# TORlN/HDR-to-SDR

Hardware: AMD Instinct MI355X
Metric: Mpixel/s HDR10->SDR (4K frames) at 1/2/4/8 GPUs; % HBM roofline (higher is better)
Workload: dtype f32

## Files before the change

hdr-to-sdr_amd/csrc/h2s_api.hip:

```cpp
#include <stdio.h>
#include <stdlib.h>

#include "h2s_host.h"

using namespace h2s::host;
using h2s::FastParams;
using h2s::KParams;

namespace {
thread_local std::string g_err;
}

namespace h2s {
namespace host {

int fail(h2s_ctx* c, int code, const std::string& msg) {
  if (c) c->err = msg;
  else g_err = msg;
  return code;
}

int hip_fail(h2s_ctx* c, hipError_t e, const char* what) {
  return fail(c, H2S_E_HIP, std::string(what) + ": " + hipGetErrorString(e));
}
// ... 129 lines not shown
  hipError_t e = hipSuccess;
  for (Event& ev : c->pend) {
    const hipError_t r = hipEventSynchronize(ev.ev);
    if (e == hipSuccess) e = r;
    c->ev_free.push_back(std::move(ev));
  }
  c->pend.clear();
  if (e != hipSuccess) return hip_fail(c, e, "draining queued launches");
  return 0;
}

int aux_stream(h2s_ctx* c, hipStream_t* out) {
  if (int rc = c->aux.get(c, "table stream")) return rc;
  *out = c->d_lut.pool = c->d_lut_yuv.pool = c->d_lut8x.pool = c->aux.s;
  return 0;
}

static hipError_t table_copy(h2s_ctx* c, void* dst, const void* src, size_t bytes) {
  hipError_t e = hipMemcpyAsync(dst, src, bytes, hipMemcpyHostToDevice, c->aux.s);
  return e == hipSuccess ? hipStreamSynchronize(c->aux.s) : e;
}

int upload_table(h2s_ctx* c, DevBuf& buf, const void* src, size_t bytes, const char* what) {
  if (int rc = buf.reserve(c, bytes, what)) return rc;
  hipError_t e = table_copy(c, buf.p, src, bytes);
  return e == hipSuccess ? 0 : hip_fail(c, e, (std::string(what) + " upload").c_str());
}

int note_launch(h2s_ctx* c, hipStream_t s) {
  if (c->pend.size() >= 32) {
    size_t j = 0;
    for (size_t i = 0; i < c->pend.size(); i++) {
      if (hipEventQuery(c->pend[i].ev) == hipSuccess) c->ev_free.push_back(std::move(c->pend[i]));
      else c->pend[j++] = std::move(c->pend[i]);
    }
    c->pend.resize(j);
  }
  Event ev;
  if (!c->ev_free.empty()) {
    ev = std::move(c->ev_free.back());
    c->ev_free.pop_back();
  }
  if (int rc = ev.get(c, "launch event")) return rc;
  hipError_t e = hipEventRecord(ev.ev, s);
  if (e != hipSuccess) {
    c->ev_free.push_back(std::move(ev));
    return hip_fail(c, e, "launch event");
  }
  c->pend.push_back(std::move(ev));
  return 0;
}

int queued_exit(h2s_ctx* c, hipStream_t s, int rc) {
  const std::string msg = c->err;
  if (note_launch(c, s) != 0) (void)hipStreamSynchronize(s);
  c->err = msg;
  return rc;
}

static int ensure_lut8x(h2s_ctx* c, hipStream_t s) {
  if (c->d_lut8x && c->lut8x_ok) return 0;
  hipStream_t aux;
  bool grew = false;
  int rc;
  if ((rc = aux_stream(c, &aux)) || (rc = c->d_lut8x.reserve(c, sizeof(unsigned) << 24, "lut3d 8-bit table", &grew)))
    return rc;
  if (grew && hipStreamSynchronize(aux) != hipSuccess) {
    c->d_lut8x.release();
    return fail(c, H2S_E_OOM, "lut3d 8-bit table allocation failed");
  }
  hipError_t e = h2s::build_lut8x(c->d_lut, c->lut_n, c->d_lut8x, s);
  if (e != hipSuccess) return hip_fail(c, e, "lut3d 8-bit table build");
  if ((rc = c->lut_built.mark(c, s, "lut3d 8-bit table build"))) return rc;
  c->lut8x_ok = true;
  return 0;
}

static int ensure_lut_yuv(h2s_ctx* c, const KParams& k, hipStream_t s) {
  int rc;
  if ((rc = c->lut_built.wait(c, s, "lattice build ordering"))) return rc;
  if (k.rgba8) return ensure_lut8x(c, s);
  if (c->d_lut_yuv && c->lut_yuv_scale == k.qscale && c->lut_yuv_rgb == k.rgba8) return 0;
  const size_t cnt = (size_t)c->lut_n * c->lut_n * c->lut_n;
  const size_t pad = 12 * (1 + (size_t)c->lut_n + (size_t)c->lut_n * c->lut_n) + 16;
  hipStream_t aux;
  bool grew = false;
  if ((rc = aux_stream(c, &aux)) || (rc = c->d_lut_yuv.reserve(c, cnt * 3 * sizeof(float) + pad, "YUV lattice", &grew)))
    return rc;
  if (grew) {
    hipError_t e = hipMemsetAsync(c->d_lut_yuv + cnt * 3, 0, pad, aux);
    if (e == hipSuccess) e = hipStreamSynchronize(aux);
    if (e != hipSuccess) {
      c->d_lut_yuv.release();
      return fail(c, H2S_E_OOM, "YUV lattice allocation failed");
    }
  }
  h2s::YuvLutConsts K;
  K.s = k.qscale;
  K.rgb = k.rgba8;
  for (int i = 0; i < 3; i++) K.k709[i] = k.k709[i], K.kcb[i] = k.kcb[i], K.kcr[i] = k.kcr[i];
  hipError_t e = h2s::build_lut_yuv(c->d_lut, c->d_lut_yuv, c->lut_n, K, s);
  if (e != hipSuccess) return hip_fail(c, e, "YUV lattice build");
  if ((rc = c->lut_built.mark(c, s, "YUV lattice build"))) return rc;
  c->lut_yuv_scale = k.qscale;
  c->lut_yuv_rgb = k.rgba8;
  return 0;
}

int prepare(h2s_ctx* c, KParams* k, bool need_lut) {
  if (!c->params_set) return fail(c, H2S_E_INVALID_ARG, "h2s_set_params was not called");
  if (need_lut && c->params.lut_enabled && !c->d_lut)
    return fail(c, H2S_E_LUT_MISSING, "lut_enabled but no LUT loaded (h2s_set_lut)");
  *k = c->k;
  k->lut = c->d_lut;
  k->lut_n = c->lut_n;
  k->lut_sg = c->lut_n;
  k->lut_sb = c->lut_n * c->lut_n;
  k->lut_max = (float)(c->lut_n - 1);
  k->eq_lut = c->d_eq;
  k->dovi = c->dovi_n ? (const h2s::DoviRec*)c->d_dovi : nullptr;
  k->dovi_n = c->dovi_n, k->dovi_f0 = 0;
  return 0;
}

KParams frame_range(const KParams& k, int f0, int n) {
  KParams kf = k;
  for (int p = 0; p < 3; p++) {
    kf.in[p] += (long long)f0 * kf.in_fp[p];
    kf.out[p] += (long long)f0 * kf.out_fp[p];
  }
  kf.nframes = n;
  kf.total = (long long)n * kf.ch * kf.ngx;
  kf.dovi_f0 += f0;
  return kf;
}

static int tiled_width(const KParams& k) { return k.W & ~(h2s::TBW - 1); }

static h2s::TileKey tile_key_of(const KParams& k, bool dbg) {
  return h2s::tile_key(k, k.in_cstep == 2 || k.out_cstep == 2, dbg);
}

hipError_t launch_tiles(const h2s_ctx* c, const KParams& k, const Route& r, const TileOpts& o) {
  FastParams F;
  resolve_fast(c, k, &F);
  for (int p = 0; p < 3; p++) {
    F.in[p] = k.in[p], F.in_ls[p] = k.in_ls[p], F.in_fp[p] = k.in_fp[p];
    F.out[p] = k.out[p], F.out_ls[p] = k.out_ls[p], F.out_fp[p] = k.out_fp[p];
  }
  F.W = tiled_width(k), F.H = k.H, F.cw = k.cw, F.ch = k.ch;
  F.icw = k.icw, F.ich = k.ich;
  F.chroma_edge = k.chroma_edge;
  F.in_semi = k.in_cstep == 2, F.in_sh = k.in_sh, F.out_semi = k.out_cstep == 2, F.out_sh = k.out_sh;
  for (int p = 0; p < 3; p++) {
    const long long ib = (long long)(p ? k.ich : k.H) * k.in_ls[p], ob = (long long)(p ? k.ch : k.H) * k.out_ls[p];
    F.in_bytes[p] = (int)(ib < 0x7fffffff ? ib : 0x7fffffff);
    F.out_bytes[p] = (int)(ob < 0x7fffffff ? ob : 0x7fffffff);
  }
  F.nbx = (unsigned)(F.W / h2s::TBW);
  F.nby = (unsigned)((k.H + h2s::TBH - 1) / h2s::TBH);
  F.nframes = (unsigned)k.nframes;
  F.tpb = c->tiles_per_block;
  F.cv_frames = o.cv_frames;
  F.dbg = o.dbg_out;
  F.dbg_stage = o.dbg;
  F.dbg_w = k.W;
  F.dbg_lut = c->d_lut;
  F.inv_nm1 = 1.0f / (float)(c->lut_n - 1);
  F.chr444 = o.chr444;
  F.chr_w = k.W;
  F.inv_c56 = 1.0f / F.c56;
  F.dovi = k.dovi, F.dovi_n = k.dovi_n, F.dovi_f0 = k.dovi_f0;
  if (k.dovi) {
// ... 533 lines not shown
```

hdr-to-sdr_amd/csrc/h2s_fast.hip:

```cpp
#include <hip/hip_runtime.h>

#include "h2s_tile_sets.h"

H2S_TILE_UNIT(fast)

namespace h2s {

__global__ void k_build_lut_yuv(const float4* rgb, float* yuv, int n3, const YuvLutConsts K) {
  const int i = blockIdx.x * 256 + threadIdx.x;
  if (i >= n3) return;
  const float4 c = rgb[i];
  const float R = clamp01(c.x), G = clamp01(c.y), B = clamp01(c.z);
  const float Y = K.k709[0] * R + K.k709[1] * G + K.k709[2] * B;
  const float cb = K.kcb[0] * R + K.kcb[1] * G + K.kcb[2] * B;
  const float cr = K.kcr[0] * R + K.kcr[1] * G + K.kcr[2] * B;
  const float s = K.s;
  if (K.rgb) {
    yuv[3 * i] = c.x, yuv[3 * i + 1] = c.y, yuv[3 * i + 2] = c.z;
    return;
  }
  constexpr float Y_ROUND = 0.0f;
  yuv[3 * i] = (16.0f + 219.0f * Y) * s + Y_ROUND;
  yuv[3 * i + 1] = 224.0f * s * 0.25f * cb;
  yuv[3 * i + 2] = 224.0f * s * 0.25f * cr;
}

TileKey tile_key(const KParams& k, bool semi, bool dbg) {
  TileKey t;
  t.trc = k.dovi ? 2 : k.transfer;
  t.tm = k.tonemap;
  t.lp = k.pipe == PIPE_LIBPLACEBO ? 1 : 0;
  t.desat = !k.desat_on ? 0 : (k.lr == 1.0f && k.lg == 1.0f && k.lb == 1.0f ? 2 : 1);
  if (t.tm == 7 || t.tm == 8 || t.lp) t.desat = 0;
  t.dbg = dbg ? 1 : 0;
  t.sub = k.vco ? 3 : k.sub;
  t.semi = semi || t.sub ? 1 : 0;
  return t;
}

namespace {

struct TileSet {
  int dbg, lp, semi, sub, family;
  hipError_t (*launch)(const FastParams&, const TileKey&, dim3, size_t, hipStream_t);
};
const TileSet SETS[] = {
#define S(UNIT, DBG, LP, SEMI, SUB, FAMILY) {DBG, LP, SEMI, SUB, FAMILY_##FAMILY, launch_set<SET_##UNIT>},
    H2S_TILE_SETS(S)
#undef S
};

const TileSet* set_of(const TileKey& k) {
  for (const TileSet& r : SETS)
    if (r.dbg == k.dbg && r.lp == k.lp && r.semi == k.semi && r.sub == k.sub && family_case(r.family, k)) return &r;
  return nullptr;
}

}

bool tile_instance(const TileKey& k) { return set_of(k) != nullptr; }

hipError_t launch_fast(const FastParams& F, const TileKey& k, hipStream_t s) {
  const long long nt = (long long)F.nbx * F.nby * F.nframes;
  if (nt == 0) return hipSuccess;
  const long long nb = (nt + F.tpb - 1) / F.tpb;
  dim3 grid((unsigned)nb);
  const size_t lds = ((size_t)F.eq_n * sizeof(uint16_t) + 15) & ~(size_t)15;
  const TileSet* set = set_of(k);
  return set ? set->launch(F, k, grid, lds, s) : hipErrorInvalidValue;
}

hipError_t build_lut_yuv(const float4* rgb, float* yuv, int n, const YuvLutConsts& K, hipStream_t st) {
  const int n3 = n * n * n;
  hipLaunchKernelGGL(k_build_lut_yuv, dim3((n3 + 255) / 256), dim3(256), 0, st, rgb, yuv, n3, K);
  return hipGetLastError();
}

}
```

hdr-to-sdr_amd/csrc/h2s_host.h:

```cpp
#pragma once
#include <hip/hip_runtime.h>
#include <math.h>
#include <stdint.h>
#include <string.h>

#include <algorithm>
#include <string>
#include <vector>

#define H2S_PRIVATE_TEST_HOOKS
#include "../../include/h2s.h"
#include "h2s_launch.h"
#include "h2s_params.h"
#include "h2s_peak.h"
#include "h2s_srcprev.h"

#pragma GCC visibility push(hidden)

namespace h2s {
namespace host {

constexpr int kEvRing = 256;
constexpr int kMaxChunks = 8;

// ... 72 lines not shown
    std::swap(ev, o.ev);
    return *this;
  }
  ~Event() {
    if (ev) hipEventDestroy(ev);
  }
  int get(h2s_ctx* c, const char* what, unsigned flags = hipEventDisableTiming) {
    if (ev) return 0;
    hipError_t e = hipEventCreateWithFlags(&ev, flags);
    if (e == hipSuccess) return 0;
    ev = nullptr;
    return hip_fail(c, e, what);
  }
};

struct Ordered {
  Event ev;
  bool pending = false;
  int wait(h2s_ctx* c, hipStream_t s, const char* what) {
    if (!pending) return 0;
    if (hipEventQuery(ev.ev) == hipSuccess) {
      pending = false;
      return 0;
    }
    hipError_t e = hipStreamWaitEvent(s, ev.ev, 0);
    return e == hipSuccess ? 0 : hip_fail(c, e, what);
  }
  int mark(h2s_ctx* c, hipStream_t s, const char* what) {
    if (int rc = ev.get(c, what)) return rc;
    hipError_t e = hipEventRecord(ev.ev, s);
    if (e != hipSuccess) return hip_fail(c, e, what);
    pending = true;
    return 0;
  }
  int sync_host(h2s_ctx* c, const char* what) {
    if (!pending) return 0;
    hipError_t e = hipEventSynchronize(ev.ev);
    if (e != hipSuccess) return hip_fail(c, e, what);
    pending = false;
    return 0;
  }
};

struct ScaleTaps {
  enum Axis { X, Y, CX, CY };
  int W = 0, H = 0, ow = 0, oh = 0;
  int T[4] = {0, 0, 0, 0};
  size_t woff[4] = {0, 0, 0, 0}, soff[4] = {0, 0, 0, 0};
  std::vector<float> w;
  std::vector<int> s;
  Dev<float> d_w;
  Dev<int> d_s;
  long long uploads = 0;
  const float* wt(int a) const { return d_w + woff[a]; }
  const int* st(int a) const { return d_s + soff[a]; }
};

}
}

struct h2s_ctx {
  int device = 0;
  h2s_params params{};
  bool params_set = false;
  h2s::KParams k{};
  h2s::host::Stream aux;
  h2s::host::Dev<float4> d_lut;
  int lut_n = 0;
  bool lut_unit = false;
  h2s::host::Dev<float> d_lut_yuv;
  float lut_yuv_scale = -1.0f;
  int lut_yuv_rgb = 0;
  h2s::host::Dev<unsigned> d_lut8x;
  bool lut8x_ok = false;
  h2s::host::Ordered lut_built;
  bool fast_enabled = true;
  bool lp_exact = false;
  h2s::host::Format in_fmt = h2s::host::PLANAR_420, out_fmt = h2s::host::PLANAR_420;
  h2s::host::Dev<h2s::DoviRec> d_dovi;
  int dovi_n = 0;
  bool dovi_tile = false;
  int peak_blocks = h2s::PEAK_BLOCKS;
  bool serial_host = false;
  int tiles_per_block = 8;
  h2s::host::Dev<uint16_t> d_eq;
  h2s::host::Dev<float4> d_pq;
  h2s::host::Dev<float4> d_hlg;
  h2s::host::Dev<float4> d_pqi;
  h2s::host::Dev<uint8_t> d_stage;
  h2s::host::Dev<uint8_t> d_prev;
  h2s::host::Dev<float2> d_stats;
  int stats_nf = 0;
  h2s::host::Dev<double2> d_fstat;
  h2s::host::Dev<h2s::CurveConsts> d_curve;
  h2s::host::Dev<h2s::PeakState> d_pk;
  h2s::host::Ordered peak_use;
  int peak_chunk = 0;
  h2s::host::Stream pk_s[2];
  std::vector<h2s::host::Event> pk_ev;
  std::string err;
  bool fail_after_launch = false;
  bool timing = false;
  h2s::host::Event ev0[h2s::host::kEvRing], ev1[h2s::host::kEvRing];
  long long ev_count = 0;
  h2s::host::Stream ps[3];
  h2s::host::Event pev[2 * h2s::host::kMaxChunks + 2];
  std::vector<h2s::host::Event> pend, ev_free;
  h2s::host::Dev<float2> d_chr;
  h2s::host::Ordered chr_use;
  h2s::host::Dev<uint8_t> d_scale;
  h2s::host::ScaleTaps scale_taps;
  h2s::host::Ordered scale_use;
};

namespace h2s {
namespace host {

struct DeviceGuard {
  int prev = -1;
  explicit DeviceGuard(int dev) {
    if (hipGetDevice(&prev) != hipSuccess) prev = -1;
    if (prev != dev) hipSetDevice(dev);
  }
  ~DeviceGuard() {
    int cur = -1;
    if (prev >= 0 && hipGetDevice(&cur) == hipSuccess && cur != prev) hipSetDevice(prev);
  }
};

struct Route {
  int path;
  bool vec, out8;
  Format in_fmt, out_fmt;
  hipStream_t s;
  bool tile() const { return path == H2S_PATH_TILE || path == H2S_PATH_TILE_TAIL; }
  Route on(hipStream_t other) const {
    Route r = *this;
    r.s = other;
    return r;
  }
};

struct TileOpts {
  const CurveConsts* cv_frames = nullptr;
  int dbg = 0;
  float* dbg_out = nullptr;
  float2* chr444 = nullptr;
};

enum Columns { COLUMNS_ALL, COLUMNS_RAGGED };


struct SourceConsts {
  double y_scale, y_off, y_black;
  double c_scale, c_off, mid;
  double m_rcr, m_gcb, m_gcr, m_bcb;
};
SourceConsts source_consts(int bits, bool full, int matrix = H2S_SRC_MATRIX_BT2020NC);
void source_kparams(KParams* k, int bits, bool full);

int validate_params(h2s_ctx* c, const h2s_params* p);
void resolve(const h2s_params* p, KParams* k, std::vector<uint16_t>* eq);
void resolve_fast(const h2s_ctx* c, const KParams& k, FastParams* F);
void build_pqi_table(std::vector<float4>* out);
void build_pq_table(double scale, std::vector<float4>* out);
void build_hlg_table(std::vector<float4>* out);
void chroma_taps(float* wx7, float* wy8);
// ... 41 lines not shown
```

hdr-to-sdr_amd/csrc/h2s_params.h:

```cpp
#pragma once
#include <hip/hip_runtime.h>
#include <stdint.h>

namespace h2s {

struct CurveConsts;

struct DoviCurve {
  int num_pivots;
  float pivots[9];
  int method[8];
  float poly[8][3];
  int mmr_order[8];
  float mmr_const[8];
  float mmr[8][3][7];
};
struct DoviRec {
  float off[3], nl[9], lin[9];
  DoviCurve comp[3];
};

struct KParams {
  int W, H, cw, ch, ngx;
  int nframes;
  long long total;
  const uint8_t* in[3];
  long long in_ls[3], in_fp[3];
  uint8_t* out[3];
  long long out_ls[3], out_fp[3];
  int in_cstep, in_sh, out_cstep, out_sh;
  float y_scale, y_off, c_scale, c_off;
  float m_rcr, m_gcb, m_gcr, m_bcb;
  float lin_scale;
  int transfer;
  int tonemap;
  int desat_on;
  float desat, lr, lg, lb;
  float lin_k;
  float gam_inv_peak, gam_inv_param, gam_low_k;
  float clip_k;
  float hable_peak_inv;
  float rein_p, rein_k;
  float mob_j, mob_a, mob_b, mob_k;
  float b_srcmin, b_range, b_inv_range, b_ks, b_inv_1mks, b_maxlum;
  float npl_1e4, e4_npl;
  float sp_srcmin, sp_srcmax, sp_kin, sp_kout, sp_pa, sp_pb, sp_qa, sp_qb, sp_qc, sp_dmin, sp_dmax;
  float sp_contrast;
  double peak;
  float b_minlum, b_bp, b_gain;
  double t_black, t_white, knee_off;
  int pipe, rgba8;
  float enc_ainv, enc_b;
  float enc_a;
  int lp_ipt;
  float lp_qs, lp_qo;
  int lp_dith;
  unsigned in_mask;
  double pd_smoothing, pd_scene_low, pd_scene_high, pd_percentile, pd_min;
  double ipt_r2l[9], ipt_l2r[9];
  double ipt_npl, ipt_os, ipt_tw;
  int lp_norm;
  float n_peak, n_nw;
  float n_rein_off, n_rein_scale, n_hable_inv, n_mob_j, n_mob_a, n_mob_b, n_mob_scale;
  int lut_enabled, lut_n, lut_sg, lut_sb;
  float lut_max;
  const float4* lut;
  float m709[9];
  int qmax, shift_out;
  float qscale;
  int eq_identity;
  const uint16_t* eq_lut;
  int chroma_edge;
  int lut_in16;
  int dither;
  int expand_rep;
  float k709[3], kcb[3], kcr[3];
  int gx0;
  float2* chr444;
  const CurveConsts* cv;
  double x_peak, x_avg, x_npl, x_tm_param;
  int x_sh;
  int sub, icw, ich;
  int full, vco;
  const DoviRec* dovi;
  int dovi_n, dovi_f0;
};

constexpr int PIPE_CPU = 1, PIPE_LIBPLACEBO = 2;

struct CurveConsts {
  float b_srcmin, b_range, b_inv_range, b_ks, b_inv_1mks, b_maxlum;
  float b_minlum, b_bp, b_gain;
  float b_e1a, b_e1b, b_ta, b_tb, b_c3, b_c2, b_c1, b_c0, b_lr, b_lc, b_thr;
  float sp_srcmin, sp_srcmax, sp_kin, sp_kout, sp_pa, sp_pb, sp_qa, sp_qb, sp_qc, sp_dmin, sp_dmax;
  float sp_qa_u, sp_qb_u, sp_qc_u, sp_pa_u, sp_pb_u, sp_k_u, sp_umin, sp_umax;
  float b_bk_a, b_bk_b, b_bk_c, b_bk_d;
  float n_peak, n_rein_off, n_rein_scale, n_hable_inv, n_mob_j, n_mob_a, n_mob_b, n_mob_scale;
  double x_peak, x_avg;
};

struct FastParams : CurveConsts {
  int W, H, cw, ch;
  int chroma_edge;
  unsigned nbx, nby, nframes;
  int tpb;
  const uint8_t* in[3];
  long long in_ls[3], in_fp[3];
  uint8_t* out[3];
  long long out_ls[3], out_fp[3];
  int in_bytes[3], out_bytes[3];
  float ys, k_r, k_g, k_b;
  float a_rv[2], a_gv[2], a_gu[2], a_bu[2];
  float log2_lin_scale;
  float log2_pq_scale;
  float y_off_c, c_mid;
  float lr, lg, lb, desat;
  float rein_p, rein_k;
  float hable_peak_inv;
  float hable_ka, hable_kb;
  float mob_j, mob_a, mob_b, mob_k;
  float npl_1e4, e4_npl;
  float tw_fold;
  float b_e1min;
  float lp_k1, lp_k2, lp_xmax, nm1, inv255, qscale, c56;
  float k709[3], kcb[3], kcr[3];
  int lp_ipt;
  float lp_qs_f, lp_qo;
  int lp_dith;
  unsigned in_mask2;
  float lp_ky[3], lp_kcb[3], lp_kcr[3], lp_cy;
  float ipt_r2l[9], ipt_l2r[9];
  const float4* pqi_tab;
  int lut_off;
  float m709[9];
  float n_nw, tw_1e4;
  const CurveConsts* cv_frames;
  float log2_nm1, s_max, stride_g, stride_b;
  float x_max;
  int og, ob, cr, cg, cb, c111;
  const float* lut_yuv;
  int lut_bytes;
  const unsigned* lut8x;
  const uint16_t* eq_lut;
  int eq_n;
  float c_bias;
  int shift_out, out8;
  int rep_rs;
  int dither;
  float2* chr444;
  int chr_w;
  float inv_c56;
  float safe_y, safe_c;
  const float4* pq_tab;
  float* dbg;
  int dbg_w;
  const float4* dbg_lut;
  float inv_nm1;
  int in_semi, in_sh, out_semi, out_sh;
  int icw, ich;
  int dbg_stage;
  const DoviRec* dovi;
  int dovi_n, dovi_f0;
  float dv_cs, dv_cm;
};

constexpr int TBW = 64, TBH = 32;
constexpr int PQ_SEG = 128;
constexpr int PQ_NSEG = 240;
constexpr float PQ_EMAX = 1.875f;
constexpr int PQI_OCT0 = -64;
constexpr int PQI_PER_OCT = 8;
constexpr int PQI_NSEG = 78 * PQI_PER_OCT;
constexpr int PQI_NTAB = PQI_NSEG + 1;

struct YuvLutConsts {
  float s, k709[3], kcb[3], kcr[3];
  int rgb;
};

}
```

hdr-to-sdr_amd/csrc/h2s_resolve.hip:

```cpp
#include "h2s_host.h"
#include "h2s_math.h"

using namespace h2s::host;
using h2s::FastParams;
using h2s::KParams;

namespace h2s {
namespace host {

int validate_params(h2s_ctx* c, const h2s_params* p) {
  if (p->transfer_in != H2S_TRC_PQ && p->transfer_in != H2S_TRC_HLG)
    return fail(c, H2S_E_INVALID_ARG, "transfer_in must be PQ or HLG");
  if (p->bits_in != 10 && p->bits_in != 12)
    return fail(c, H2S_E_UNSUPPORTED, "bits_in must be 10 or 12 (yuv420p10le / yuv420p12le)");
  if (p->bits_out != 8 && p->bits_out != 10 && p->bits_out != 12)
    return fail(c, H2S_E_UNSUPPORTED, "bits_out must be 8, 10 or 12");
  if (p->tonemap < H2S_TM_NONE || p->tonemap > H2S_TM_SPLINE)
    return fail(c, H2S_E_INVALID_ARG, "unknown tonemap operator");
  if (p->tonemap == H2S_TM_SPLINE && !isnan(p->tm_param) && !(p->tm_param >= 0.0 && p->tm_param <= 1.5))
    return fail(c, H2S_E_INVALID_ARG, "spline contrast (tm_param) must be in [0, 1.5]");
  if (p->mode != H2S_MODE_COMPAT8 && p->mode != H2S_MODE_NATIVE)
    return fail(c, H2S_E_INVALID_ARG, "mode must be COMPAT8 or NATIVE");
  if (p->desat_luma < 0 || p->desat_luma > 2) return fail(c, H2S_E_INVALID_ARG, "unknown desat_luma");
  if (!(p->gamma > 0) || !isfinite(p->gamma)) return fail(c, H2S_E_INVALID_ARG, "gamma must be > 0");
// ... 280 lines not shown
    const double num = fmax(xp - c1, 0.0), den = c2 - c3 * xp;
    return den > 0 ? pow(num / den, 1.0 / m1) * scale : HUGE_VAL;
  }, out);
}

void build_hlg_table(std::vector<float4>* out) {
  const double a = 0.17883277, b = 0.28466892, c = 0.55991073;
  build_seg_table([&](double e) {
    if (!(e > 0)) return 0.0;
    return e <= 0.5 ? e * e / 3.0 : (exp((e - c) / a) + b) / 12.0;
  }, out);
}

void resolve_fast(const h2s_ctx* c, const KParams& k, FastParams* F) {
  memset(F, 0, sizeof(*F));
  const h2s_params* p = &c->params;
  const int sh = p->bits_in - 8;
  const SourceConsts sc = source_consts(p->bits_in, k.full != 0);
  const double ys = sc.y_scale, yo = sc.y_off, cs = sc.c_scale, co = sc.c_off;
  const double mrcr = sc.m_rcr, mgcb = sc.m_gcb, mgcr = sc.m_gcr, mbcb = sc.m_bcb;
  F->ys = (float)ys;
  F->k_r = (float)(yo + mrcr * co);
  F->k_g = (float)(yo + (mgcb + mgcr) * co);
  F->k_b = (float)(yo + mbcb * co);
  F->y_off_c = (float)yo;
  F->c_mid = (float)sc.mid;
  for (int odd = 0; odd < 2; odd++) {
    const double d = odd ? 8.0 : 4.0;
    F->a_rv[odd] = (float)(mrcr * cs / d);
    F->a_gu[odd] = (float)(mgcb * cs / d);
    F->a_gv[odd] = (float)(mgcr * cs / d);
    F->a_bu[odd] = (float)(mbcb * cs / d);
  }
  F->log2_lin_scale = (float)log2((p->transfer_in == H2S_TRC_HLG ? 1000.0 : 10000.0) / p->npl);
  F->log2_pq_scale = (float)log2(10000.0 / p->npl);
  {
    const bool table = p->transfer_in == H2S_TRC_PQ || k.pipe != h2s::PIPE_LIBPLACEBO;
    const double amax = std::max(std::max(fabs(mrcr), fabs(mgcb) + fabs(mgcr)), fabs(mbcb)) * cs;
    const double safe_c = k.full ? floor(((double)h2s::PQ_EMAX - 1e-3 - (1.0 + 1e-4)) / amax) : (double)(112 << sh);
    const double ymax = k.full ? 1.0 + 1e-4 : (double)h2s::PQ_EMAX - amax * safe_c - 1e-3;
    F->safe_c = table ? (float)safe_c : HUGE_VALF;
    F->safe_y = table ? (float)(ymax * h2s::PQ_SEG + 1.0) : HUGE_VALF;
  }
  F->lr = k.lr, F->lg = k.lg, F->lb = k.lb, F->desat = k.desat;
  F->rein_p = k.rein_p, F->rein_k = k.rein_k;
  F->hable_peak_inv = k.hable_peak_inv;
  F->hable_ka = (float)(2.1 / 15.0 * (double)k.hable_peak_inv);
  F->hable_kb = (float)(0.25 / 15.0 * (double)k.hable_peak_inv);
  F->mob_j = k.mob_j, F->mob_a = k.mob_a, F->mob_b = k.mob_b, F->mob_k = k.mob_k;
  F->npl_1e4 = k.npl_1e4, F->e4_npl = k.e4_npl;
  F->b_e1min = (float)h2s::hd_pq_encode(1e-6 * p->npl / 10000.0);
  F->tw_fold = (float)(p->npl / k.t_white);
  F->lp_k1 = (float)(log2((double)k.enc_ainv) / 2.4 + log2(255.0));
  F->lp_k2 = (float)(255.0 * (double)k.enc_b);
  F->lp_xmax = (float)(pow(1.0 + (double)k.enc_b, 2.4) / (double)k.enc_ainv * 1.001);
  F->nm1 = (float)(c->lut_n - 1);
  F->inv255 = 1.0f / 255.0f;
  F->qscale = k.qscale;
  F->c56 = 56.0f * k.qscale;
  for (int i = 0; i < 3; i++) F->k709[i] = k.k709[i], F->kcb[i] = k.kcb[i], F->kcr[i] = k.kcr[i];
  F->lp_ipt = k.lp_ipt;
  F->lp_qs_f = k.lp_qs / 255.0f;
  F->lp_qo = k.lp_qo;
  for (int i = 0; i < 3; i++) {
    F->lp_ky[i] = (float)((double)k.k709[i] / 255.0 * 219.0 * (double)k.qscale);
    F->lp_kcb[i] = (float)((double)k.kcb[i] / 255.0 * 56.0 * (double)k.qscale);
    F->lp_kcr[i] = (float)((double)k.kcr[i] / 255.0 * 56.0 * (double)k.qscale);
  }
  F->lp_cy = 16.0f * k.qscale + 0.5f;
  F->lp_dith = k.lp_dith;
  F->in_mask2 = k.in_mask | (k.in_mask << 16);
  for (int i = 0; i < 9; i++)
    F->ipt_r2l[i] = (float)(k.ipt_r2l[i] * k.ipt_npl), F->ipt_l2r[i] = (float)(k.ipt_l2r[i] * (p->npl / k.t_white));
  F->pqi_tab = c->d_pqi;
  F->lut_off = k.lut_enabled ? 0 : 1;
  F->n_nw = k.n_nw;
  F->tw_1e4 = (float)(k.t_white / 10000.0);
  for (int i = 0; i < 9; i++) F->m709[i] = k.m709[i];
  h2s::curve_fast(k, static_cast<h2s::CurveConsts*>(F));
  const int n = c->lut_n;
  F->log2_nm1 = (float)log2((double)(n - 1));
  F->s_max = nextafterf((float)(n - 1), 0.0f);
  F->x_max = 0.999999f;
  F->stride_g = (float)(12 * n);
  F->stride_b = (float)(12 * n * n);
  F->og = 12 * n;
  F->ob = 12 * n * n;
  F->c111 = 12 * (1 + n + n * n);
  F->cr = F->c111 - 12;
  F->cg = F->c111 - F->og;
  F->cb = F->c111 - F->ob;
  F->lut_yuv = c->d_lut_yuv;
  F->lut_bytes = 12 * n * n * n;
  F->lut8x = c->d_lut8x;
  F->eq_lut = c->d_eq;
  F->eq_n = k.qmax + 1;
  F->c_bias = 128.0f * k.qscale + 0.5f;
  F->shift_out = k.shift_out;
  F->rep_rs = k.expand_rep && k.shift_out ? 8 - k.shift_out : 31;
  F->dither = k.dither;
  F->out8 = p->bits_out == 8 ? 1 : 0;
  F->pq_tab = p->transfer_in == H2S_TRC_HLG && k.pipe != h2s::PIPE_LIBPLACEBO ? c->d_hlg : c->d_pq;
}


static double bicubic(double x) {
  const double B = 0.0, C = 0.6;
  x = fabs(x);
  if (x < 1.0) return ((12 - 9 * B - 6 * C) * x * x * x + (-18 + 12 * B + 6 * C) * x * x + (6 - 2 * B)) / 6.0;
  if (x < 2.0) return ((-B - 6 * C) * x * x * x + (6 * B + 30 * C) * x * x + (-12 * B - 48 * C) * x + (8 * B + 24 * C)) / 6.0;
  return 0.0;
}

void chroma_taps(float* wx7, float* wy8) {
  double tx[7], ty[8], sx = 0, sy = 0;
  for (int i = 0; i < 7; i++) sx += (tx[i] = bicubic((i - 3) / 2.0));
  for (int j = 0; j < 8; j++) sy += (ty[j] = bicubic((j - 3.5) / 2.0));
  for (int i = 0; i < 7; i++) wx7[i] = (float)(tx[i] / sx);
  for (int j = 0; j < 8; j++) wy8[j] = (float)(ty[j] / sy);
}

int resize_taps(int src, int dst, std::vector<float>* w, std::vector<int>* start) {
  const double scale = (double)src / dst, fw = scale > 1.0 ? scale : 1.0;
  const int T = (int)ceil(4.0 * fw) + 1;
  const size_t w0 = w->size(), s0_ = start->size();
  w->resize(w0 + (size_t)dst * T, 0.0f);
  start->resize(s0_ + dst, 0);
  for (int o = 0; o < dst; o++) {
    const double c = (o + 0.5) * scale - 0.5;
    const int s0 = (int)floor(c - 2.0 * fw) + 1;
    double sum = 0.0, tmp[128];
    for (int i = 0; i < T && i < 128; i++) sum += (tmp[i] = bicubic((s0 + i - c) / fw));
    for (int i = 0; i < T && i < 128; i++) (*w)[w0 + (size_t)o * T + i] = (float)(tmp[i] / sum);
    (*start)[s0_ + o] = s0;
  }
  return T;
}

PeakModel peak_model(const h2s_ctx* c, const KParams& k) {
  h2s::PeakModel m;
  m.t_white = k.t_white, m.t_black = k.t_black, m.knee_off = k.knee_off;
  m.contrast = k.sp_contrast, m.tm_param = c->params.tm_param, m.static_peak = k.peak;
  m.smoothing = k.pd_smoothing, m.scene_low = k.pd_scene_low, m.scene_high = k.pd_scene_high;
  m.percentile = k.pd_percentile, m.min_peak = k.pd_min;
  m.iir_a = k.pd_smoothing > 0.0 ? 1.0 - exp(-1.0 / k.pd_smoothing) : 1.0;
  m.npx = (double)k.W * k.H;
  m.nblocks = c->peak_blocks;
  m.pct = k.pd_percentile < 100.0 ? 1 : 0;
  m.family = k.tonemap;
  m.pq = h2s::pq_refs(k.t_white, k.t_black);
  return m;
}

}
}
```

hdr-to-sdr_amd/csrc/h2s_tile.h:

```cpp
#pragma once
#include "h2s_tile_io.h"

namespace h2s {

__device__ __forceinline__ CurveConsts curve_of(const CurveConsts* frames, int f) {
  typedef __attribute__((address_space(4))) const float cfloat;
  constexpr int n = (int)(sizeof(CurveConsts) / sizeof(float));
  cfloat* src = (cfloat*)frames + __builtin_amdgcn_readfirstlane(f) * n;
  CurveConsts r;
  float* dst = reinterpret_cast<float*>(&r);
#pragma unroll
  for (int i = 0; i < n; i++) dst[i] = src[i];
  return r;
}

constexpr int TILE_WPE = 5;
constexpr int TILE_WPE_LP = TILE_WPE;

template <int TRC, int TM, int DESAT, int LP, int DBG = 0, bool SEMI = false, int SUB = 0>
__global__ __launch_bounds__(256) __attribute__((amdgpu_waves_per_eu(LP ? TILE_WPE_LP : TILE_WPE))) void k_tile(
    const FastParams F) {
  static_assert(DBG == 0 || DBG == 1, "the stage is F.dbg_stage, not a template value");
  static_assert(SUB == 0 || SUB == 3 || (LP == 0 && DBG == 0), "4:2:2 / 4:4:4 input: CPU chain product instances only");
  static_assert(SUB != 3 || (DBG == 0 && SEMI), "top-left 4:2:0 input: the SEMI product instances");
  constexpr bool S420 = SUB == 0 || SUB == 3;
  constexpr int YST = row_stride<LP>(), HST = YST;
  static_assert(TBH * C422_ST <= (CBH + 2) * HST && TBH * C444_ST <= 2 * (CBH + 2) * HST, "hrow holds the SUB windows");
  __shared__ __attribute__((aligned(16))) unsigned char yin[YIN_BYTES];
  __shared__ float hrow[2][(CBH + 2) * HST];
  __shared__ float csum[2][CBH * CBW];
  __shared__ float4 pq_lds[PQ_NSEG + 1];
  __shared__ float4 pqi_lds[LP ? PQI_NTAB : 1];
  extern __shared__ uint16_t eq_lds[];
  __shared__ int tflag[2];
  __shared__ int offtab[4];
  __shared__ unsigned spread_lds[LP ? 256 : 1];
  constexpr int ESC = TRC == 0 || !LP ? PQ_SEG : 1;

  const int t = threadIdx.x;
  const int lane = t & 63, w = t >> 6;
  const unsigned ntiles = F.nbx * F.nby * F.nframes;
  unsigned tile = (unsigned)xcd_remap(blockIdx.x, gridDim.x) * (unsigned)F.tpb;
  const unsigned tend = tile + (unsigned)F.tpb < ntiles ? tile + (unsigned)F.tpb : ntiles;

  TileGeo geo = tile_geo(F, tile);
  const LaneOfs lofs = lane_ofs<SEMI>(F, t);
  TileRegs<SEMI, SUB> cur = tile_load<SEMI, SUB>(F, geo, t, lofs);
  const __amdgpu_buffer_rsrc_t req = __builtin_amdgcn_make_buffer_rsrc((void*)F.eq_lut, (short)0, 2 * F.eq_n, 0x00020000);
  const unsigned eq0 = __builtin_amdgcn_raw_buffer_load_b16(req, 2 * t, 0, 0);
  float4 pq0 = make_float4(0.0f, 0.0f, 0.0f, 0.0f);
  const bool stage_pq = TRC != 1 || !LP || F.lp_ipt;
  if (stage_pq && t < PQ_NSEG) {
    const __amdgpu_buffer_rsrc_t rpq = __builtin_amdgcn_make_buffer_rsrc((void*)F.pq_tab, (short)0, 16 * PQ_NSEG, 0x00020000);
    pq0 = __builtin_bit_cast(float4, __builtin_amdgcn_raw_buffer_load_b128(rpq, 16 * t, 0, 0));
  }
  const int eq_sh = SEMI ? F.out_sh : 0;
  if (t < F.eq_n) eq_lds[t] = (uint16_t)(((eq0 << F.shift_out) | (eq0 >> F.rep_rs)) << eq_sh);
  for (int i = t + 256; i < F.eq_n; i += 256) {
    const unsigned v = __builtin_amdgcn_raw_buffer_load_b16(req, 2 * i, 0, 0);
    eq_lds[i] = (uint16_t)(((v << F.shift_out) | (v >> F.rep_rs)) << eq_sh);
  }
  if (stage_pq && t < PQ_NSEG)
    pq_lds[t + 1] = (TRC == 0 || LP) && t == 0 ? make_float4(0.0f, 0.0f, 3.40282347e38f, 0.0f) : pq0;
  if (stage_pq && t == 255) pq_lds[0] = make_float4(0.0f, 0.0f, 0.0f, 0.0f);
  if (t < 2) tflag[t] = 0;
  if (t < 3) offtab[t] = t == 0 ? 12 : (t == 1 ? F.og : F.ob);
  if (LP) {
    unsigned x = (unsigned)t;
    x = (x | (x << 8)) & 0x0F00Fu;
    x = (x | (x << 4)) & 0x0C30C3u;
    spread_lds[t] = (x | (x << 2)) & 0x249249u;
  }
  __syncthreads();
  if (LP && (F.lp_ipt || TRC == 2)) {
    const __amdgpu_buffer_rsrc_t rpi = __builtin_amdgcn_make_buffer_rsrc((void*)F.pqi_tab, (short)0, 16 * PQI_NTAB, 0x00020000);
    for (int i = t; i < PQI_NTAB; i += 256)
      pqi_lds[i] = __builtin_bit_cast(float4, __builtin_amdgcn_raw_buffer_load_b128(rpi, 16 * i, 0, 0));
  }

  const int qx = (lane >> 2) & 3, qy = lane >> 4, pxl = lane & 1, pyl = (lane >> 1) & 1;
  const int xl = 16 * w + 2 * qx + pxl, yl = 2 * qy + pyl;
  uint16_t* ybase = reinterpret_cast<uint16_t*>(yin + luma_at(xl, yl));
  const float* h0 = hrow[0] + (qy + 1) * HST + xl;
  const float* h1 = hrow[1] + (qy + 1) * HST + xl;
  const int hb = SUB == 3 ? (pyl ? HST : 0) : (pyl ? HST : -HST);
  const float* c0 = hrow[0] + yl * C422_ST + (xl >> 1);
  const float* c1 = hrow[1] + yl * C422_ST + (xl >> 1);
  const int16_t* s0 = reinterpret_cast<const int16_t*>(hrow[0]) + yl * C444_ST + xl;
  const int16_t* s1 = reinterpret_cast<const int16_t*>(hrow[1]) + yl * C444_ST + xl;
  float* csb = csum[0] + qy * CBW + 8 * w + qx;

  const float yoff = in_vgpr(F.y_off_c) * (float)ESC + (ESC == PQ_SEG ? 1.0f : 0.0f);
  const float cmid = in_vgpr(F.c_mid);
  const float a_rv = in_vgpr(F.a_rv[1]) * (float)ESC, a_gv = in_vgpr(F.a_gv[1]) * (float)ESC,
              a_gu = in_vgpr(F.a_gu[1]) * (float)ESC, a_bu = in_vgpr(F.a_bu[1]) * (float)ESC;
  const float stride_g = in_vgpr(F.stride_g), stride_b = in_vgpr(F.stride_b);
  const int og = in_vgpr(F.og), ob = in_vgpr(F.ob), ocr = in_vgpr(F.cr), ocg = in_vgpr(F.cg), ocb = in_vgpr(F.cb);
  const float log2_nm1 = in_vgpr(F.log2_nm1), x_max = in_vgpr(F.x_max);
  const float ysc = in_vgpr(F.ys) * (float)ESC;
  const float ydq = F.dither ? dither_off(xl, yl) - 0.5f : 0.0f;
  const StepK K{a_rv, a_gv, a_gu, a_bu, stride_g, stride_b, og, ob, ocr, ocg, ocb, log2_nm1, x_max,
                TM == 5 && !LP ? in_vgpr(F.hable_kb) : F.hable_kb, F.c111, rintf(1.0f / F.inv_nm1), offtab,
                LP ? in_vgpr(F.lp_k2) : 0.0f, LP ? in_vgpr(F.lp_k2 + 255.0f) : 0.0f, LP ? F.lp_cy + ydq : 0.0f,
                LP ? in_vgpr(F.lp_k1) : 0.0f};
  gu32* lut8v = LP ? in_vgpr64(F.lut8x) : nullptr;
  float qo[4];
#pragma unroll
  for (int i = 0; i < 4; i++)
    qo[i] = LP ? F.lp_qo + (F.lp_dith ? bayer16(xl + 8 * (i & 1), yl + 8 * (i >> 1)) : 0.5f) -
                     (F.lut_off ? 0.0f : F.lp_k2 * F.lp_qs_f)
               : 0.5f;

  auto steps = [&](const TileGeo& g, auto fast) {
    constexpr bool FB = decltype(fast)::value;
    constexpr int YR2 = YROW / 2;
    if constexpr (FB) {
      H2S_MARK("body: fast");
    } else {
      H2S_MARK("body: exact-capable");
    }
    CurveConsts cv = F;
    if ((TM == 7 || TM == 8 || LP) && F.cv_frames) cv = curve_of(F.cv_frames, g.f);
    const CDoviRec* const dv =
        TRC == 2 ? (const CDoviRec*)F.dovi + __builtin_amdgcn_readfirstlane(F.dovi_n == 1 ? 0 : F.dovi_f0 + g.f) : nullptr;
    if constexpr (LP && TM == 7) {
      cv.b_e1b = in_vgpr(cv.b_e1b), cv.b_tb = in_vgpr(cv.b_tb), cv.b_c2 = in_vgpr(cv.b_c2);
      cv.b_lc = in_vgpr(cv.b_lc), cv.b_bk_b = in_vgpr(cv.b_bk_b), cv.b_bk_d = in_vgpr(cv.b_bk_d);
    } else if constexpr (LP && TM == 8) {
      cv.sp_qb_u = in_vgpr(cv.sp_qb_u), cv.sp_pb_u = in_vgpr(cv.sp_pb_u);
      cv.sp_srcmax = in_vgpr(cv.sp_srcmax), cv.sp_umax = in_vgpr(cv.sp_umax);
    }
    const __amdgpu_buffer_rsrc_t lut = __builtin_amdgcn_make_buffer_rsrc((void*)F.lut_yuv, (short)0, F.lut_bytes, 0x00020000);
    const int live = !FB && DBG == 0 && !F.chr444 ? F.H - g.py0 : TBH;
    auto chroma_out = [&](int s, float oyv, float ozv) {
      if (!FB && F.chr444) {
        const int px = g.px0 + xl + 8 * (s & 1), py = g.py0 + yl + 8 * (s >> 1);
        F.chr444[(long long)py * F.chr_w + px] = make_float2(oyv * F.inv_c56, ozv * F.inv_c56);
        return;
      }
      H2S_MARK("S6 chroma quad sums");
      const int oc = 4 * (s >> 1) * CBW + 4 * (s & 1);
      const float su = quad_sum(oyv), sv = quad_sum(ozv);
      csb[oc] = su;
      csb[oc + CBH * CBW] = sv;
    };
    if constexpr (LP && DBG == 0) {
      if (!F.lut_off) {
        unsigned vp = 0;
#pragma unroll
// ... 134 lines not shown
```

hdr-to-sdr_amd/csrc/h2s_tile_px.h:

```cpp
#pragma once
#include "h2s_tile_tone.h"


namespace h2s {

typedef float f3 __attribute__((ext_vector_type(3)));

typedef unsigned u2v __attribute__((ext_vector_type(2)));
typedef unsigned u4v __attribute__((ext_vector_type(4)));

typedef __attribute__((address_space(1))) const unsigned gu32;
__device__ __forceinline__ gu32* in_vgpr64(const unsigned* x) {
  gu32* y;
  asm volatile("v_mov_b64 %0, %1" : "=v"(y) : "s"((gu32*)x));
  return y;
}

struct StepK {
  float a_rv, a_gv, a_gu, a_bu;
  float stride_g, stride_b;
  int og, ob, ocr, ocg, ocb;
  float log2_nm1, x_max;
  float hable_kb;
  int c111;
// ... 120 lines not shown
      const bool safe2 = to_linear<TRC, ESC, NOEX, true>(F, pq_lds, er, eg, eb, r, gg, bl);
      tone<TRC, TM, DESAT, LP, true>(F, cv, pq_lds, pqi_lds, r, gg, bl, safe2, emax_s, K.hable_kb, luma);
    }
  }
}

__device__ __forceinline__ unsigned lp_table_read(const FastParams& F, const StepK& K, gu32* lut8v,
                                                  const unsigned* spread_lds, float r, float gg, float bl,
                                                  float qoff) {
  auto q8 = [&](float x) -> unsigned {
    const float e = fexp2(fmaf(flog2(__builtin_amdgcn_fmed3f(x, 0.0f, F.lp_xmax)), 1.0f / 2.4f, K.lp_k1));
    return (unsigned)fmaf(__builtin_amdgcn_fmed3f(e, K.lp_k2, K.lp_hi), F.lp_qs_f, qoff);
  };
  unsigned idx;
  const unsigned qr = q8(r), qg = q8(gg), qb = q8(bl);
  H2S_MARK("S4 lut3d table read");
  asm("v_lshl_or_b32 %0, %1, 1, %2" : "=v"(idx) : "v"(spread_lds[qb]), "v"(spread_lds[qg]));
  asm("v_lshl_or_b32 %0, %1, 1, %2" : "=v"(idx) : "v"(idx), "v"(spread_lds[qr]));
  return lut8v[idx];
}

__device__ __forceinline__ f3 lp_ycbcr(const FastParams& F, const StepK& K, float R8, float G8, float B8) {
  f3 o;
  o.x = fmaf(F.lp_ky[0], R8, fmaf(F.lp_ky[1], G8, fmaf(F.lp_ky[2], B8, K.lp_cy)));
  o.y = fmaf(F.lp_kcb[0], R8, fmaf(F.lp_kcb[1], G8, F.lp_kcb[2] * B8));
  o.z = fmaf(F.lp_kcr[0], R8, fmaf(F.lp_kcr[1], G8, F.lp_kcr[2] * B8));
  return o;
}

template <int TRC, int TM, int DESAT, int LP, int DBG, bool NOEX = false>
__device__ __forceinline__ unsigned px_chain(const FastParams& F, const CurveConsts& cv, const float4* pq_lds,
                                             const float4* pqi_lds, const uint16_t* eq_lds, gu32* lut8v, const unsigned* spread_lds,
                                             __amdgpu_buffer_rsrc_t lut, const StepK K, float ybs, float U, float V,
                                             long long di, float& oyv, float& ozv, float qoff, float ydq,
                                             const CDoviRec* dv = nullptr) {
  constexpr bool EQM = !LP;
  const long long dpl = (long long)F.dbg_w * F.H;
  auto dput = [&](float a, float b_, float c) {
    if (di >= 0) F.dbg[di] = a, F.dbg[dpl + di] = b_, F.dbg[2 * dpl + di] = c;
  };
  float r, gg, bl;
  lin_tone<TRC, TM, DESAT, LP, DBG, NOEX>(F, cv, pq_lds, pqi_lds, K, ybs, U, V, dput, r, gg, bl, dv);
  H2S_MARKV("S3 encode", r, gg, bl);
  if (DBG && F.dbg_stage == 2) dput(r, gg, bl);
  f3 o;
  if (LP && F.lut_off) {
    auto enc = [&](float x) -> float {
      const float e = fexp2(fmaf(flog2(__builtin_amdgcn_fmed3f(x, 0.0f, F.lp_xmax)), 1.0f / 2.4f, F.lp_k1)) - F.lp_k2;
      return __builtin_amdgcn_fmed3f(e, 0.0f, 255.0f);
    };
    const float R = enc(F.m709[0] * r + F.m709[1] * gg + F.m709[2] * bl);
    const float G = enc(F.m709[3] * r + F.m709[4] * gg + F.m709[5] * bl);
    const float B = enc(F.m709[6] * r + F.m709[7] * gg + F.m709[8] * bl);
    if (DBG && (F.dbg_stage == 3 || F.dbg_stage == 4)) dput(R * F.inv255, G * F.inv255, B * F.inv255);
    o.x = fmaf(F.lp_ky[0], R, fmaf(F.lp_ky[1], G, fmaf(F.lp_ky[2], B, K.lp_cy)));
    o.y = fmaf(F.lp_kcb[0], R, fmaf(F.lp_kcb[1], G, F.lp_kcb[2] * B));
    o.z = fmaf(F.lp_kcr[0], R, fmaf(F.lp_kcr[1], G, F.lp_kcr[2] * B));
  } else if constexpr (LP) {
    if (DBG && F.dbg_stage == 3) {
      auto ev = [&](float x) {
        const float e = fexp2(fmaf(flog2(__builtin_amdgcn_fmed3f(x, 0.0f, F.lp_xmax)), 1.0f / 2.4f, F.lp_k1)) - F.lp_k2;
        return __builtin_amdgcn_fmed3f(e, 0.0f, 255.0f) * F.inv255;
      };
      dput(ev(r), ev(gg), ev(bl));
    }
    const unsigned v = lp_table_read(F, K, lut8v, spread_lds, r, gg, bl, qoff);
    const float R8 = (float)(v & 255u), G8 = (float)((v >> 8) & 255u), B8 = (float)((v >> 16) & 255u);
    H2S_MARK("S5 Y'CbCr");
    if (DBG && F.dbg_stage == 4) dput(R8 * F.inv255, G8 * F.inv255, B8 * F.inv255);
    o = lp_ycbcr(F, K, R8, G8, B8);
  } else {
    float cr, cg, cb, dr, dg, db;
    {
      float sr, sg, sb;
      sr = __builtin_amdgcn_fmed3f(fexp2(flog2(r) * (1.0f / 2.4f)), 0.0f, 1.0f) * K.nm1;
      sg = __builtin_amdgcn_fmed3f(fexp2(flog2(gg) * (1.0f / 2.4f)), 0.0f, 1.0f) * K.nm1;
      sb = __builtin_amdgcn_fmed3f(fexp2(flog2(bl) * (1.0f / 2.4f)), 0.0f, 1.0f) * K.nm1;
      asm("" : "+v"(sr), "+v"(sg), "+v"(sb));
      H2S_MARKV("S4a cell, fractions", sr, sg, sb);
      dr = __builtin_amdgcn_fractf(sr), dg = __builtin_amdgcn_fractf(sg), db = __builtin_amdgcn_fractf(sb);
      cr = sr - dr, cg = sg - dg, cb = sb - db;
    }
    H2S_MARKV("S4b tetrahedron select", dr, dg, db);
    const int base = (int)fmaf(cb, K.stride_b, fmaf(cg, K.stride_g, cr * 12.0f));
    int om, ocn;
    float dmax, dmin, dmid;
    unsigned umin = 0, amax = 0;
    {
      const unsigned ur = __builtin_bit_cast(unsigned, dr) & ~15u;
      const unsigned ug = (__builtin_bit_cast(unsigned, dg) & ~15u) | 5u;
      const unsigned ub = (__builtin_bit_cast(unsigned, db) & ~15u) | 10u;
      unsigned umax, umid;
      asm("v_max3_u32 %0, %1, %2, %3" : "=v"(umax) : "v"(ur), "v"(ug), "v"(ub));
      asm("v_min3_u32 %0, %1, %2, %3" : "=v"(umin) : "v"(ur), "v"(ug), "v"(ub));
      asm("v_med3_u32 %0, %1, %2, %3" : "=v"(umid) : "v"(ur), "v"(ug), "v"(ub));
      amax = umax & 12u;
      const unsigned amin = umin & 12u;
      om = *reinterpret_cast<const int*>(reinterpret_cast<const char*>(K.offtab) + amax);
      ocn = K.c111 - *reinterpret_cast<const int*>(reinterpret_cast<const char*>(K.offtab) + amin);
      dmax = __builtin_bit_cast(float, umax), dmin = __builtin_bit_cast(float, umin), dmid = __builtin_bit_cast(float, umid);
    }
    H2S_MARKV("S4c weights, uniformity, gathers, blend", dmax, dmid, dmin);
    const float w0 = 1.0f - dmax, w1 = dmax - dmid, w2 = dmid - dmin, w3 = dmin;
    auto blend = [&](const f3 c0, const f3 c1, const f3 c2, const f3 c3) {
      f3 r = w0 * c0 + w1 * c1 + w2 * c2 + w3 * c3;
      r.x = fmaf(w3, c3.x, fmaf(w2, c2.x, fmaf(w1, c1.x, fmaf(w0, c0.x, ydq))));
      return r;
    };
    bool step_uniform;
    int b0, m0, n0;
    {
      unsigned tkey, key;
      asm("v_and_or_b32 %0, %1, 3, %2" : "=v"(tkey) : "v"(umin), "v"(amax));
      asm("v_lshl_or_b32 %0, %1, 4, %2" : "=v"(key) : "v"(base), "v"(tkey));
      const unsigned key0 = __builtin_amdgcn_readfirstlane(key);
      step_uniform = __builtin_amdgcn_ballot_w64(key != key0) == 0;
      b0 = 0, m0 = 0, n0 = 0;
      if (step_uniform) {
        b0 = (int)(key0 >> 4);
        m0 = __builtin_amdgcn_readfirstlane(om), n0 = __builtin_amdgcn_readfirstlane(ocn);
      }
    }
    if (step_uniform) {
      typedef __attribute__((address_space(4))) const float cfl;
      cfl* L = (cfl*)F.lut_yuv;
      auto sl = [&](int off) {
        const int i = off >> 2;
        return f3{L[i], L[i + 1], L[i + 2]};
      };
      o = blend(sl(b0), sl(b0 + m0), sl(b0 + n0), sl(b0 + F.c111));
    } else {
      o = blend(__builtin_amdgcn_raw_buffer_load_b96(lut, base, 0, 0), __builtin_amdgcn_raw_buffer_load_b96(lut, base + om, 0, 0),
                __builtin_amdgcn_raw_buffer_load_b96(lut, base + ocn, 0, 0),
                __builtin_amdgcn_raw_buffer_load_b96(lut, base, F.c111, 0));
    }
    if (DBG && F.dbg_stage == 3) dput((cr + dr) * F.inv_nm1, (cg + dg) * F.inv_nm1, (cb + db) * F.inv_nm1);
    if (DBG && F.dbg_stage == 4) {
      const float4 q0 = F.dbg_lut[base / 12], q1 = F.dbg_lut[(base + om) / 12], q2 = F.dbg_lut[(base + ocn) / 12],
                   q3 = F.dbg_lut[(base + F.c111) / 12];
      dput(w0 * q0.x + w1 * q1.x + w2 * q2.x + w3 * q3.x, w0 * q0.y + w1 * q1.y + w2 * q2.y + w3 * q3.y,
           w0 * q0.z + w1 * q1.z + w2 * q2.z + w3 * q3.z);
    }
  }
  H2S_MARKV("S7 eq", o.x, o.y, o.z);
  if (DBG && F.dbg_stage == 5) dput(o.x - (EQM ? 0.0f : 0.5f) - ydq, 4.0f * o.y, 4.0f * o.z);
  oyv = o.y, ozv = o.z;
  if constexpr (EQM) {
    const unsigned qb = __builtin_bit_cast(unsigned, o.x + 8388608.0f);
    unsigned off;
    asm("v_lshlrev_b16 %0, 1, %1" : "=v"(off) : "v"(qb));
    return *reinterpret_cast<const uint16_t*>(reinterpret_cast<const char*>(eq_lds) + off);
  } else {
    return eq_lds[(int)o.x];
  }
}

__device__ __forceinline__ float quad_sum(float v) {
  v += __builtin_bit_cast(float, __builtin_amdgcn_update_dpp(0, __builtin_bit_cast(int, v), 0xB1, 0xF, 0xF, false));
  return v + __builtin_bit_cast(float, __builtin_amdgcn_update_dpp(0, __builtin_bit_cast(int, v), 0x4E, 0xF, 0xF, false));
}

template <class T>
__device__ __forceinline__ T in_vgpr(T x) {
  T y;
  asm volatile("v_mov_b32 %0, %1" : "=v"(y) : "s"(x));
  return y;
}

}
```

Before: 276,900.

## Parameterize LUT record stride and auto-select tiles per block from CU count

```diff
diff --git a/hdr-to-sdr_amd/csrc/h2s_api.hip b/hdr-to-sdr_amd/csrc/h2s_api.hip
--- a/hdr-to-sdr_amd/csrc/h2s_api.hip
+++ b/hdr-to-sdr_amd/csrc/h2s_api.hip
@@ -235,13 +235,14 @@
   if (k.rgba8) return ensure_lut8x(c, s);
   if (c->d_lut_yuv && c->lut_yuv_scale == k.qscale && c->lut_yuv_rgb == k.rgba8) return 0;
   const size_t cnt = (size_t)c->lut_n * c->lut_n * c->lut_n;
-  const size_t pad = 12 * (1 + (size_t)c->lut_n + (size_t)c->lut_n * c->lut_n) + 16;
+  constexpr size_t REC = h2s::LUT_REC, REC_F = h2s::LUT_REC_F;
+  const size_t pad = REC * (1 + (size_t)c->lut_n + (size_t)c->lut_n * c->lut_n) + 16;
   hipStream_t aux;
   bool grew = false;
-  if ((rc = aux_stream(c, &aux)) || (rc = c->d_lut_yuv.reserve(c, cnt * 3 * sizeof(float) + pad, "YUV lattice", &grew)))
+  if ((rc = aux_stream(c, &aux)) || (rc = c->d_lut_yuv.reserve(c, cnt * REC + pad, "YUV lattice", &grew)))
     return rc;
   if (grew) {
-    hipError_t e = hipMemsetAsync(c->d_lut_yuv + cnt * 3, 0, pad, aux);
+    hipError_t e = hipMemsetAsync(c->d_lut_yuv + cnt * REC_F, 0, pad, aux);
     if (e == hipSuccess) e = hipStreamSynchronize(aux);
     if (e != hipSuccess) {
       c->d_lut_yuv.release();
diff --git a/hdr-to-sdr_amd/csrc/h2s_fast.hip b/hdr-to-sdr_amd/csrc/h2s_fast.hip
--- a/hdr-to-sdr_amd/csrc/h2s_fast.hip
+++ b/hdr-to-sdr_amd/csrc/h2s_fast.hip
@@ -15,14 +15,16 @@
   const float cb = K.kcb[0] * R + K.kcb[1] * G + K.kcb[2] * B;
   const float cr = K.kcr[0] * R + K.kcr[1] * G + K.kcr[2] * B;
   const float s = K.s;
+  float* rec = yuv + (size_t)LUT_REC_F * i;
+  for (int j = 3; j < LUT_REC_F; j++) rec[j] = 0.0f;
   if (K.rgb) {
-    yuv[3 * i] = c.x, yuv[3 * i + 1] = c.y, yuv[3 * i + 2] = c.z;
+    rec[0] = c.x, rec[1] = c.y, rec[2] = c.z;
     return;
   }
   constexpr float Y_ROUND = 0.0f;
-  yuv[3 * i] = (16.0f + 219.0f * Y) * s + Y_ROUND;
-  yuv[3 * i + 1] = 224.0f * s * 0.25f * cb;
-  yuv[3 * i + 2] = 224.0f * s * 0.25f * cr;
+  rec[0] = (16.0f + 219.0f * Y) * s + Y_ROUND;
+  rec[1] = 224.0f * s * 0.25f * cb;
+  rec[2] = 224.0f * s * 0.25f * cr;
 }
 
 TileKey tile_key(const KParams& k, bool semi, bool dbg) {
@@ -60,9 +62,23 @@
 
 bool tile_instance(const TileKey& k) { return set_of(k) != nullptr; }
 
-hipError_t launch_fast(const FastParams& F, const TileKey& k, hipStream_t s) {
-  const long long nt = (long long)F.nbx * F.nby * F.nframes;
+constexpr int TPB_DEFAULT = 8, TPB_WHOLE = 12;
+static int auto_tpb(long long ntiles, int lp) {
+  static int cus[64];
+  int dev = 0;
+  if (hipGetDevice(&dev) != hipSuccess || dev < 0 || dev >= 64) return TPB_DEFAULT;
+  if (cus[dev] == 0 && hipDeviceGetAttribute(&cus[dev], hipDeviceAttributeMultiprocessorCount, dev) != hipSuccess)
+    cus[dev] = -1;
+  if (cus[dev] <= 0) return TPB_DEFAULT;
+  const long long resident = (long long)cus[dev] * (lp ? 4 : TILE_WPE);
+  return ntiles % (resident * TPB_WHOLE) == 0 ? TPB_WHOLE : TPB_DEFAULT;
+}
+
+hipError_t launch_fast(const FastParams& F0, const TileKey& k, hipStream_t s) {
+  const long long nt = (long long)F0.nbx * F0.nby * F0.nframes;
   if (nt == 0) return hipSuccess;
+  FastParams F = F0;
+  if (F.tpb <= 0) F.tpb = auto_tpb(nt, k.lp);
   const long long nb = (nt + F.tpb - 1) / F.tpb;
   dim3 grid((unsigned)nb);
   const size_t lds = ((size_t)F.eq_n * sizeof(uint16_t) + 15) & ~(size_t)15;
diff --git a/hdr-to-sdr_amd/csrc/h2s_host.h b/hdr-to-sdr_amd/csrc/h2s_host.h
--- a/hdr-to-sdr_amd/csrc/h2s_host.h
+++ b/hdr-to-sdr_amd/csrc/h2s_host.h
@@ -178,7 +178,7 @@
   bool dovi_tile = false;
   int peak_blocks = h2s::PEAK_BLOCKS;
   bool serial_host = false;
-  int tiles_per_block = 8;
+  int tiles_per_block = 0;
   h2s::host::Dev<uint16_t> d_eq;
   h2s::host::Dev<float4> d_pq;
   h2s::host::Dev<float4> d_hlg;
diff --git a/hdr-to-sdr_amd/csrc/h2s_params.h b/hdr-to-sdr_amd/csrc/h2s_params.h
--- a/hdr-to-sdr_amd/csrc/h2s_params.h
+++ b/hdr-to-sdr_amd/csrc/h2s_params.h
@@ -99,6 +99,10 @@
   double x_peak, x_avg;
 };
 
+constexpr int LUT_REC = 12;
+constexpr int LUT_REC_F = LUT_REC / (int)sizeof(float);
+static_assert(LUT_REC % 4 == 0 && LUT_REC >= 12, "a record holds three floats");
+
 struct FastParams : CurveConsts {
   int W, H, cw, ch;
   int chroma_edge;
diff --git a/hdr-to-sdr_amd/csrc/h2s_resolve.hip b/hdr-to-sdr_amd/csrc/h2s_resolve.hip
--- a/hdr-to-sdr_amd/csrc/h2s_resolve.hip
+++ b/hdr-to-sdr_amd/csrc/h2s_resolve.hip
@@ -386,16 +386,17 @@
   F->log2_nm1 = (float)log2((double)(n - 1));
   F->s_max = nextafterf((float)(n - 1), 0.0f);
   F->x_max = 0.999999f;
-  F->stride_g = (float)(12 * n);
-  F->stride_b = (float)(12 * n * n);
-  F->og = 12 * n;
-  F->ob = 12 * n * n;
-  F->c111 = 12 * (1 + n + n * n);
-  F->cr = F->c111 - 12;
+  constexpr int REC = h2s::LUT_REC;
+  F->stride_g = (float)(REC * n);
+  F->stride_b = (float)(REC * n * n);
+  F->og = REC * n;
+  F->ob = REC * n * n;
+  F->c111 = REC * (1 + n + n * n);
+  F->cr = F->c111 - REC;
   F->cg = F->c111 - F->og;
   F->cb = F->c111 - F->ob;
   F->lut_yuv = c->d_lut_yuv;
-  F->lut_bytes = 12 * n * n * n;
+  F->lut_bytes = REC * n * n * n;
   F->lut8x = c->d_lut8x;
   F->eq_lut = c->d_eq;
   F->eq_n = k.qmax + 1;
diff --git a/hdr-to-sdr_amd/csrc/h2s_tile.h b/hdr-to-sdr_amd/csrc/h2s_tile.h
--- a/hdr-to-sdr_amd/csrc/h2s_tile.h
+++ b/hdr-to-sdr_amd/csrc/h2s_tile.h
@@ -64,7 +64,7 @@
     pq_lds[t + 1] = (TRC == 0 || LP) && t == 0 ? make_float4(0.0f, 0.0f, 3.40282347e38f, 0.0f) : pq0;
   if (stage_pq && t == 255) pq_lds[0] = make_float4(0.0f, 0.0f, 0.0f, 0.0f);
   if (t < 2) tflag[t] = 0;
-  if (t < 3) offtab[t] = t == 0 ? 12 : (t == 1 ? F.og : F.ob);
+  if (t < 3) offtab[t] = t == 0 ? LUT_REC : (t == 1 ? F.og : F.ob);
   if (LP) {
     unsigned x = (unsigned)t;
     x = (x | (x << 8)) & 0x0F00Fu;
diff --git a/hdr-to-sdr_amd/csrc/h2s_tile_px.h b/hdr-to-sdr_amd/csrc/h2s_tile_px.h
--- a/hdr-to-sdr_amd/csrc/h2s_tile_px.h
+++ b/hdr-to-sdr_amd/csrc/h2s_tile_px.h
@@ -226,7 +226,7 @@
       cr = sr - dr, cg = sg - dg, cb = sb - db;
     }
     H2S_MARKV("S4b tetrahedron select", dr, dg, db);
-    const int base = (int)fmaf(cb, K.stride_b, fmaf(cg, K.stride_g, cr * 12.0f));
+    const int base = (int)fmaf(cb, K.stride_b, fmaf(cg, K.stride_g, cr * (float)LUT_REC));
     int om, ocn;
     float dmax, dmin, dmid;
     unsigned umin = 0, amax = 0;
@@ -266,11 +266,14 @@
       }
     }
     if (step_uniform) {
-      typedef __attribute__((address_space(4))) const float cfl;
-      cfl* L = (cfl*)F.lut_yuv;
+      typedef float srec __attribute__((ext_vector_type(4)));
+      typedef srec __attribute__((aligned(4))) srec_a4;
+      typedef __attribute__((address_space(4))) const char cch;
+      typedef __attribute__((address_space(4))) const srec_a4 csrec;
+      cch* L = (cch*)F.lut_yuv;
       auto sl = [&](int off) {
-        const int i = off >> 2;
-        return f3{L[i], L[i + 1], L[i + 2]};
+        const srec v = *(csrec*)(L + (unsigned)off);
+        return f3{v.x, v.y, v.z};
       };
       o = blend(sl(b0), sl(b0 + m0), sl(b0 + n0), sl(b0 + F.c111));
     } else {
@@ -280,8 +283,8 @@
     }
     if (DBG && F.dbg_stage == 3) dput((cr + dr) * F.inv_nm1, (cg + dg) * F.inv_nm1, (cb + db) * F.inv_nm1);
     if (DBG && F.dbg_stage == 4) {
-      const float4 q0 = F.dbg_lut[base / 12], q1 = F.dbg_lut[(base + om) / 12], q2 = F.dbg_lut[(base + ocn) / 12],
-                   q3 = F.dbg_lut[(base + F.c111) / 12];
+      const float4 q0 = F.dbg_lut[base / LUT_REC], q1 = F.dbg_lut[(base + om) / LUT_REC],
+                   q2 = F.dbg_lut[(base + ocn) / LUT_REC], q3 = F.dbg_lut[(base + F.c111) / LUT_REC];
       dput(w0 * q0.x + w1 * q1.x + w2 * q2.x + w3 * q3.x, w0 * q0.y + w1 * q1.y + w2 * q2.y + w3 * q3.y,
            w0 * q0.z + w1 * q1.z + w2 * q2.z + w3 * q3.z);
     }
```

Result: no change. 279,200, median of 6 (+0.8%).
